# lbrndnr/LBAudioDetective

Hardware: AMD Instinct MI355X
Metric: audio_seconds_fingerprinted_per_sec (higher is better)
Workload: dtype f32; 1 GPU; configs[1]: 100k synthetic 1 s @44.1 kHz mono clips, 1024-pt FFT, stride 64, fingerprint-only, input resident in HBM; one step = 10 passes over the batch; clips_per_gpu=100000, samples_per_clip=44100, window=1024, stride=64, bands=32, subfingerprints_per_clip=5, kernel_variant=0, parallelism=clips sharded x1, no collective

## Files before the change

lbaudiodetective_amd/csrc/api_detective.cpp:

```cpp
#include "internal.hpp"

#include <new>
#include "audiofile.hpp"

#include <cmath>
#include <cstdlib>
#include <cstring>

namespace lbad {

uint64_t subfingerprint_count(uint64_t n_samples, uint32_t window, uint32_t stride) {
    if (stride == 0 || n_samples < window) return 0;
    return ((n_samples - window) / stride) / kRowsPerFrame;
}

static bool valid_window(uint32_t w) { return w >= kMinWindow && w <= kMaxWindow && (w & (w - 1)) == 0; }

static void free_plan(Plan& p) {
    if (p.d_tw) (void)hipFree(p.d_tw);
    if (p.d_bands) (void)hipFree(p.d_bands);
    if (p.d_bin_const) (void)hipFree(p.d_bin_const);
    if (p.d_claim) (void)hipFree(p.d_claim);
    p = Plan();
}

static OSStatus plan_kernels(Plan& p) {
    p.pruned_ok = rows_pruned_supported(p);
    if (p.pruned_ok && !p.d_bin_const) {
        std::vector<float> bc;
        rows_pruned_constants(bc);
        LBAD_HIP(hipMalloc(reinterpret_cast<void**>(&p.d_bin_const), bc.size() * sizeof(float)));
        LBAD_HIP(hipMemcpy(p.d_bin_const, bc.data(), bc.size() * sizeof(float), hipMemcpyHostToDevice));
    }
    p.full_ok = rows_full_supported(p);
    p.stream_ok = rows_stream_supported(p);
    p.stream2_ok = rows_stream2_supported(p);
    if ((p.full_ok || p.stream_ok || p.stream2_ok) && !p.d_claim) LBAD_HIP(hipMalloc(reinterpret_cast<void**>(&p.d_claim), 8 * sizeof(uint32_t)));
    return noErr;
}

OSStatus ensure_plan(LBAudioDetective* d) {
    const double rate = d->format.mSampleRate;
    if (!valid_window(d->window) || d->stride == 0 || d->bands == 0 || d->bands > kMaxBands || !(rate > 0.0) ||
        d->subfp_len == 0 || d->subfp_len > LBAD_MAX_SUBFINGERPRINT_LENGTH ||
        d->subfp_len > kRowsPerFrame * d->bands)
        return kLBAudioDetectiveArgumentInvalid;
    Plan& p = d->plan;
    p.tune_waves = d->tune_waves;
    p.tune_cache = d->tune_cache;
    if (p.valid && p.sample_rate == rate && p.window == d->window && p.bands == d->bands && p.subfp_len == d->subfp_len) {
        if (p.stride == d->stride) return noErr;
        p.stride = d->stride;
        p.valid = false;
        OSStatus st = plan_kernels(p);
        if (st != noErr) return st;
        p.valid = true;
        return noErr;
    }
    if (!device_ready()) return kLBAudioDetectiveDeviceUnavailable;
    free_plan(p);
    p.tune_waves = d->tune_waves;
    p.tune_cache = d->tune_cache;
    p.sample_rate = rate;
    p.window = d->window;
    p.stride = d->stride;
    p.bands = d->bands;
    p.subfp_len = d->subfp_len;
    p.log2w = 0;
    while ((1u << p.log2w) < p.window) ++p.log2w;
    p.keep = (p.subfp_len + 1) / 2;
    make_band_table(rate, p.window, p.bands, p.table);
    std::vector<float> re, im;
    make_twiddles(p.window, re, im);
    const size_t half = p.window / 2;
    LBAD_HIP(hipMalloc(reinterpret_cast<void**>(&p.d_tw), 2 * half * sizeof(float)));
    LBAD_HIP(hipMemcpy(p.d_tw, re.data(), half * sizeof(float), hipMemcpyHostToDevice));
    LBAD_HIP(hipMemcpy(p.d_tw + half, im.data(), half * sizeof(float), hipMemcpyHostToDevice));
    plan_sparse(p);
    std::vector<uint32_t> tbl(8 * (size_t)p.bands + 1);
    for (uint32_t b = 0; b < p.bands; ++b) {
        tbl[b] = p.table.lo[b];
        tbl[p.bands + b] = p.table.hi[b];
        const float div = (float)(p.table.indices[b + 1] - p.table.indices[b]);
        std::memcpy(&tbl[2 * p.bands + b], &div, 4);
        tbl[3 * p.bands + b] = p.bands;
        tbl[4 * p.bands + b] = b;
        uint32_t mult = 0, off = 0xFFFFFFFFu;
        if (p.sparse.ok) {
            const uint32_t pos = b >= 16 ? p.sparse.pos_right[b - 16] : (b == p.sparse.left ? p.sparse.pos_left : 0xFFu);
            if (pos != 0xFFu) { mult = p.sparse.n_stored; off = pos; }
        }
        tbl[5 * p.bands + b] = mult;
        tbl[6 * p.bands + b] = off;
        tbl[7 * p.bands + b] = p.table.term_at[b];
    }
    tbl[8 * (size_t)p.bands] = p.table.term_end;
    LBAD_HIP(hipMalloc(reinterpret_cast<void**>(&p.d_bands), tbl.size() * sizeof(uint32_t)));
    LBAD_HIP(hipMemcpy(p.d_bands, tbl.data(), tbl.size() * sizeof(uint32_t), hipMemcpyHostToDevice));
    OSStatus st = plan_kernels(p);
    if (st != noErr) return st;
    p.valid = true;
    return noErr;
}

static OSStatus ensure_scratch(LBAudioDetective* d, uint64_t floats) {
    if (d->d_frames_cap >= floats) return noErr;
    if (d->d_frames) (void)hipFree(d->d_frames);
    d->d_frames = nullptr;
    d->d_frames_cap = 0;
    LBAD_HIP(hipMalloc(reinterpret_cast<void**>(&d->d_frames), floats * sizeof(float)));
    d->d_frames_cap = floats;
    return noErr;
}

static hipError_t apply_file_tail(const Plan& p, const FileTail& t, const void* d_pcm, uint64_t rows_total, float* frames,
                                  hipStream_t stream) {
    if (t.mode == 3) return launch_empty_rows_batch(p, t.d_files, t.n_files, t.max_rows, frames, stream);
    const uint64_t rows = t.rows ? t.rows : rows_total;
    if (t.first_short >= rows) return hipSuccess;
    float* file_frames = frames + t.row_begin * p.bands;
    if (t.mode == 1)
        return launch_empty_rows(p, file_frames + t.first_short * p.bands, rows - t.first_short, stream);
    if (t.mode == 2)
        return launch_file_tail(p, static_cast<const float*>(d_pcm) + t.pcm_begin, t.n_client, p.stride, t.first_short,
                                (uint32_t)(rows - t.first_short), t.d_tbl, file_frames, stream);
    return hipSuccess;
}

struct StreamOrder {
    LBAudioDetective* d;
    hipStream_t stream;
    bool active = false;
    hipError_t begin() {
        hipStreamCaptureStatus cap = hipStreamCaptureStatusNone;
        if (hipStreamIsCapturing(stream, &cap) != hipSuccess) { (void)hipGetLastError(); return hipSuccess; }
        if (cap != hipStreamCaptureStatusNone) return hipSuccess;
        if (!d->done) {
            hipError_t e = hipEventCreateWithFlags(&d->done, hipEventDisableTiming);
            if (e != hipSuccess) return e;
        }
        active = true;
        if (d->done_valid && d->done_stream != stream) return hipStreamWaitEvent(stream, d->done, 0);
        return hipSuccess;
    }
    ~StreamOrder() {
        if (!active) return;
        d->done_valid = hipEventRecord(d->done, stream) == hipSuccess;
        d->done_stream = stream;
    }
};

OSStatus fingerprint_clips_device(LBAudioDetective* d, const void* d_pcm_raw, uint32_t fmt, uint64_t n_clips,
                                  uint64_t spc, uint32_t* d_packed, float* d_raw, float* d_haar, hipStream_t stream,
                                  const FileTail* tail, size_t n_tails) {
    if (fmt > 2) return kLBAudioDetectiveArgumentInvalid;
    if (tail && (n_clips != 1 || fmt != 0)) return kLBAudioDetectiveArgumentInvalid;
    LBAD_LOCK(d);
    const size_t elem = fmt == 1 ? 2 : 4;
    const char* d_pcm = static_cast<const char*>(d_pcm_raw);
    OSStatus st = ensure_plan(d);
    if (st != noErr) return st;
    const Plan& p = d->plan;
    const uint64_t per = subfingerprint_count(spc, p.window, p.stride);
    if (per == 0 || n_clips == 0) return noErr;
    if (per > 0xFFFFFFFFull / kRowsPerFrame) return kLBAudioDetectiveArgumentInvalid;
    const bool pairs_ok = reinterpret_cast<uintptr_t>(d_pcm_raw) % (2 * elem) == 0 && ((spc & 1) == 0 || n_clips == 1);
    const bool stream_ok = p.stream_ok && pairs_ok;
    const bool stream2_ok = p.stream2_ok && pairs_ok && d->variant != 3;
    const bool full_ok = p.full_ok && rows_full_supported_fmt(p, fmt);
    bool special = p.pruned_ok || full_ok || stream_ok || stream2_ok;
    if (d->variant == 3) {
        if (!full_ok && !p.pruned_ok) return kLBAudioDetectiveArgumentInvalid;
    }
    if (d->variant == 1) special = false;
    if (d->variant >= 2 && !special) return kLBAudioDetectiveArgumentInvalid;
    StreamOrder order{d, stream};
    LBAD_HIP(order.begin());
    const bool special2 = d->variant != 1 && haar_select32_supported(p);
    const bool compact = special && p.pruned_ok && special2 && p.sparse.ok && !tail && !d_raw && d->variant != 4;
    auto stage1 = [&](const void* pcm_in, uint64_t nc, float* frames_out) -> hipError_t {
        if (special && p.pruned_ok)
            return launch_rows_pruned(p, p.d_bin_const, pcm_in, fmt, nc, spc, (uint32_t)per, frames_out, stream, compact);
        if (special && stream2_ok) return launch_rows_stream2(p, pcm_in, fmt, nc, spc, (uint32_t)per, frames_out, stream);
        if (special && full_ok) return launch_rows_full(p, pcm_in, fmt, nc, spc, (uint32_t)per, frames_out, stream);
        if (special) return launch_rows_stream(p, pcm_in, fmt, nc, spc, (uint32_t)per, frames_out, stream);
        return launch_fft_bands(p, pcm_in, fmt, nc, spc, (uint32_t)per, frames_out, stream);
    };
    auto stage2 = [&](float* frames_in, uint64_t nf, uint32_t* packed_out, float* haar_out) -> hipError_t {
        if (compact && haar_out) {
            hipError_t e = hipMemsetAsync(haar_out, 0, nf * kRowsPerFrame * p.bands * sizeof(float), stream);
            if (e != hipSuccess) return e;
        }
        return special2 ? launch_haar_select32(p, frames_in, nf, packed_out, haar_out, stream, compact)
                        : launch_haar_select(p, frames_in, nf, packed_out, haar_out, stream);
    };
    const uint64_t frame_floats = (uint64_t)kRowsPerFrame * p.bands;
    if (d_raw) {
        LBAD_HIP(stage1(d_pcm, n_clips, d_raw));
        for (size_t t = 0; tail && t < n_tails; ++t) LBAD_HIP(apply_file_tail(p, tail[t], d_pcm, per * kRowsPerFrame, d_raw, stream));
        LBAD_HIP(stage2(d_raw, n_clips * per, d_packed, d_haar));
        return noErr;
    }
    uint64_t chunk = (d->scratch_limit / sizeof(float)) / (per * frame_floats);
    if (chunk == 0) chunk = 1;
    if (chunk > n_clips) chunk = n_clips;
    st = ensure_scratch(d, chunk * per * frame_floats);
    if (st != noErr) return st;
    auto mark = [&]() -> hipError_t {
        if (!d->timing) return hipSuccess;
        if (d->ev_used == d->ev.size()) {
            hipEvent_t e;
            hipError_t err = hipEventCreate(&e);
            if (err != hipSuccess) return err;
            d->ev.push_back(e);
        }
        return hipEventRecord(d->ev[d->ev_used++], stream);
    };
    for (uint64_t c0 = 0; c0 < n_clips; c0 += chunk) {
        const uint64_t nc = (n_clips - c0) < chunk ? (n_clips - c0) : chunk;
        LBAD_HIP(mark());
        LBAD_HIP(stage1(d_pcm + c0 * spc * elem, nc, d->d_frames));
        for (size_t t = 0; tail && t < n_tails; ++t)
            LBAD_HIP(apply_file_tail(p, tail[t], d_pcm, per * kRowsPerFrame, d->d_frames, stream));
        LBAD_HIP(mark());
        LBAD_HIP(stage2(d->d_frames, nc * per, d_packed + c0 * per * kPackedWords,
                        d_haar ? d_haar + c0 * per * frame_floats : nullptr));
        LBAD_HIP(mark());
    }
    return noErr;
}

constexpr size_t kPinnedLimit = 512u << 10;

OSStatus grow_device(void** ptr, size_t* cap, size_t bytes) {
    if (*cap >= bytes) return noErr;
    if (*ptr) (void)hipFree(*ptr);
    *ptr = nullptr;
    *cap = 0;
    const size_t want = bytes + bytes / 4;
    LBAD_HIP(hipMalloc(ptr, want));
    *cap = want;
    return noErr;
}

static OSStatus ensure_io(LBAudioDetective* d, size_t pcm_bytes, size_t packed_bytes, size_t extra_bytes) {
    OSStatus st = grow_device(&d->d_io_pcm, &d->d_io_pcm_cap, pcm_bytes + extra_bytes + 256);
    if (st != noErr) return st;
// ... 751 lines not shown
```

lbaudiodetective_amd/csrc/k_haar_select32.hip:

```cpp
#include "internal.hpp"

#include <type_traits>

namespace lbad {
namespace {

constexpr uint32_t kCand = 128;
constexpr int kChunkDw = 20;

constexpr uint32_t kFastDivLo = 0x0D800000u;
constexpr uint32_t kFastDivHi = 0x7E800000u;

struct DivGuard {
    uint32_t lo = 0xFFFFFFFFu, hi = 0u;
    __device__ __forceinline__ void dividends(float a, float b) {
        lo = min(lo, min((__float_as_uint(a) << 1) - 1u, (__float_as_uint(b) << 1) - 1u));
    }
    __device__ __forceinline__ void inputs(float a, float b) {
        hi = max(hi, max(__float_as_uint(a) & 0x7fffffffu, __float_as_uint(b) & 0x7fffffffu));
    }
    __device__ __forceinline__ bool bad() const { return lo < 2u * kFastDivLo - 1u || hi > kFastDivHi; }
};

template <bool FAST>
__device__ __forceinline__ float div_c(float x, float d, float r) {
    if constexpr (FAST) {
        const float q0 = __fmul_rn(x, r);
        const float e = __fmaf_rn(-d, q0, x);
        return __fmaf_rn(e, r, q0);
    } else {
        return __fdiv_rn(x, d);
    }
}

constexpr uint32_t kHistBuckets = 2048;

__device__ __forceinline__ uint32_t wave_prefix_sum(uint32_t x) {
    x += (uint32_t)__builtin_amdgcn_update_dpp(0, (int)x, 0x111 , 0xF, 0xF, false);
    x += (uint32_t)__builtin_amdgcn_update_dpp(0, (int)x, 0x112 , 0xF, 0xF, false);
    x += (uint32_t)__builtin_amdgcn_update_dpp(0, (int)x, 0x114 , 0xF, 0xF, false);
    x += (uint32_t)__builtin_amdgcn_update_dpp(0, (int)x, 0x118 , 0xF, 0xF, false);
    x += (uint32_t)__builtin_amdgcn_update_dpp(0, (int)x, 0x142 , 0xA, 0xF, false);
    x += (uint32_t)__builtin_amdgcn_update_dpp(0, (int)x, 0x143 , 0xC, 0xF, false);
    return x;
}

template <int WAVES>
__device__ __forceinline__ uint32_t slots_sum(const uint32_t* slot) {
    uint32_t c = 0;
#pragma unroll
    for (int w = 0; w < WAVES; ++w) c += slot[w];
    return c;
}

template <int WAVES>
__device__ __forceinline__ uint32_t block_sum(uint32_t v, uint32_t* s_red, int parity) {
#pragma unroll
    for (int off = 32; off > 0; off >>= 1) v += __shfl_xor(v, off, 64);
    uint32_t* slot = s_red + 8 * parity;
    if ((threadIdx.x & 63) == 0) slot[threadIdx.x >> 6] = v;
    __syncthreads();
    return slots_sum<WAVES>(slot);
}

constexpr uint32_t kLightLo = 0x25800000u;
typedef float f2 __attribute__((ext_vector_type(2)));

struct LightGuard {
    uint32_t lo_in = 0xFFFFFFFFu, lo_4 = 0xFFFFFFFFu;
    float hi = 0.0f;
    __device__ __forceinline__ void levels34(f2 a, f2 b, f2 c) {
        auto t = [](float x) { return (__float_as_uint(x) << 1) - 1u; };
        lo_4 = min(min(min(t(a.x), t(a.y)), min(t(b.x), t(b.y))), min(t(c.x), t(c.y)));
    }
    __device__ __forceinline__ bool bad(float s4) const {
        return lo_in < 2u * kLightLo - 1u || lo_4 < 2u * kFastDivLo - 1u || !(hi <= __uint_as_float(kFastDivHi)) || s4 != s4;
    }
};

template <bool FAST>
__device__ __forceinline__ float haar16_impl(const float (&in)[16], float (&d)[15], float root, float r_root,
                                             float root2, float r_root2, DivGuard& g) {
    float a[16];
#pragma unroll
    for (int i = 0; i < 16; i += 2) {
        if constexpr (FAST) {
            g.inputs(in[i], in[i + 1]);
            g.dividends(in[i], in[i + 1]);
        }
        a[i] = div_c<FAST>(in[i], root, r_root);
        a[i + 1] = div_c<FAST>(in[i + 1], root, r_root);
    }
    auto bfly = [&](float x, float y, float& sum, float& dif) {
        const float sp = __fadd_rn(x, y), sm = __fsub_rn(x, y);
        if constexpr (FAST) g.dividends(sp, sm);
        sum = div_c<FAST>(sp, root2, r_root2);
        dif = div_c<FAST>(sm, root2, r_root2);
    };
    float s1[8], s2[4], s3[2], s4;
#pragma unroll
    for (int i = 0; i < 8; ++i) bfly(a[2 * i], a[2 * i + 1], s1[i], d[i]);
#pragma unroll
    for (int i = 0; i < 4; ++i) bfly(s1[2 * i], s1[2 * i + 1], s2[i], d[8 + i]);
#pragma unroll
    for (int i = 0; i < 2; ++i) bfly(s2[2 * i], s2[2 * i + 1], s3[i], d[12 + i]);
    bfly(s3[0], s3[1], s4, d[14]);
    return s4;
}


struct DivConst {
    unsigned long long r, nd;
    __device__ __forceinline__ explicit DivConst(float d)
        : r(__builtin_amdgcn_readfirstlane(__float_as_uint(__fdiv_rn(1.0f, d)))),
          nd(__builtin_amdgcn_readfirstlane(__float_as_uint(-d))) {}
};

__device__ __forceinline__ void pk_prescale8(f2 (&x)[8], f2 (&q)[8], const DivConst& c) {
    asm("v_pk_mul_f32 %0, %8, %[r] op_sel_hi:[1,0]\n"
        "v_pk_mul_f32 %1, %9, %[r] op_sel_hi:[1,0]\n"
        "v_pk_mul_f32 %2, %10, %[r] op_sel_hi:[1,0]\n"
        "v_pk_mul_f32 %3, %11, %[r] op_sel_hi:[1,0]\n"
        "v_pk_mul_f32 %4, %12, %[r] op_sel_hi:[1,0]\n"
        "v_pk_mul_f32 %5, %13, %[r] op_sel_hi:[1,0]\n"
        "v_pk_mul_f32 %6, %14, %[r] op_sel_hi:[1,0]\n"
        "v_pk_mul_f32 %7, %15, %[r] op_sel_hi:[1,0]\n"
        "v_pk_fma_f32 %8, %0, %[nd], %8 op_sel_hi:[1,0,1]\n"
        "v_pk_fma_f32 %9, %1, %[nd], %9 op_sel_hi:[1,0,1]\n"
        "v_pk_fma_f32 %10, %2, %[nd], %10 op_sel_hi:[1,0,1]\n"
        "v_pk_fma_f32 %11, %3, %[nd], %11 op_sel_hi:[1,0,1]\n"
        "v_pk_fma_f32 %12, %4, %[nd], %12 op_sel_hi:[1,0,1]\n"
        "v_pk_fma_f32 %13, %5, %[nd], %13 op_sel_hi:[1,0,1]\n"
        "v_pk_fma_f32 %14, %6, %[nd], %14 op_sel_hi:[1,0,1]\n"
        "v_pk_fma_f32 %15, %7, %[nd], %15 op_sel_hi:[1,0,1]\n"
        "v_pk_fma_f32 %0, %8, %[r], %0 op_sel_hi:[1,0,1]\n"
        "v_pk_fma_f32 %1, %9, %[r], %1 op_sel_hi:[1,0,1]\n"
        "v_pk_fma_f32 %2, %10, %[r], %2 op_sel_hi:[1,0,1]\n"
        "v_pk_fma_f32 %3, %11, %[r], %3 op_sel_hi:[1,0,1]\n"
        "v_pk_fma_f32 %4, %12, %[r], %4 op_sel_hi:[1,0,1]\n"
        "v_pk_fma_f32 %5, %13, %[r], %5 op_sel_hi:[1,0,1]\n"
        "v_pk_fma_f32 %6, %14, %[r], %6 op_sel_hi:[1,0,1]\n"
        "v_pk_fma_f32 %7, %15, %[r], %7 op_sel_hi:[1,0,1]\n"
        "s_nop 0"
        : "=&v"(q[0]), "=&v"(q[1]), "=&v"(q[2]), "=&v"(q[3]), "=&v"(q[4]), "=&v"(q[5]), "=&v"(q[6]), "=&v"(q[7]),
          "+v"(x[0]), "+v"(x[1]), "+v"(x[2]), "+v"(x[3]), "+v"(x[4]), "+v"(x[5]), "+v"(x[6]), "+v"(x[7])
        : [r] "s"(c.r), [nd] "s"(c.nd));
}

__device__ __forceinline__ void pk_level1(f2 (&p)[8], f2 (&q)[8], const DivConst& c) {
    asm("v_pk_add_f32 %8, %8, %8 op_sel:[0,1] op_sel_hi:[0,1] neg_hi:[0,1]\n"
        "v_pk_add_f32 %9, %9, %9 op_sel:[0,1] op_sel_hi:[0,1] neg_hi:[0,1]\n"
        "v_pk_add_f32 %10, %10, %10 op_sel:[0,1] op_sel_hi:[0,1] neg_hi:[0,1]\n"
        "v_pk_add_f32 %11, %11, %11 op_sel:[0,1] op_sel_hi:[0,1] neg_hi:[0,1]\n"
        "v_pk_add_f32 %12, %12, %12 op_sel:[0,1] op_sel_hi:[0,1] neg_hi:[0,1]\n"
        "v_pk_add_f32 %13, %13, %13 op_sel:[0,1] op_sel_hi:[0,1] neg_hi:[0,1]\n"
        "v_pk_add_f32 %14, %14, %14 op_sel:[0,1] op_sel_hi:[0,1] neg_hi:[0,1]\n"
        "v_pk_add_f32 %15, %15, %15 op_sel:[0,1] op_sel_hi:[0,1] neg_hi:[0,1]\n"
        "v_pk_mul_f32 %0, %8, %[r] op_sel_hi:[1,0]\n"
        "v_pk_mul_f32 %1, %9, %[r] op_sel_hi:[1,0]\n"
        "v_pk_mul_f32 %2, %10, %[r] op_sel_hi:[1,0]\n"
        "v_pk_mul_f32 %3, %11, %[r] op_sel_hi:[1,0]\n"
        "v_pk_mul_f32 %4, %12, %[r] op_sel_hi:[1,0]\n"
        "v_pk_mul_f32 %5, %13, %[r] op_sel_hi:[1,0]\n"
        "v_pk_mul_f32 %6, %14, %[r] op_sel_hi:[1,0]\n"
        "v_pk_mul_f32 %7, %15, %[r] op_sel_hi:[1,0]\n"
        "v_pk_fma_f32 %8, %0, %[nd], %8 op_sel_hi:[1,0,1]\n"
        "v_pk_fma_f32 %9, %1, %[nd], %9 op_sel_hi:[1,0,1]\n"
        "v_pk_fma_f32 %10, %2, %[nd], %10 op_sel_hi:[1,0,1]\n"
        "v_pk_fma_f32 %11, %3, %[nd], %11 op_sel_hi:[1,0,1]\n"
        "v_pk_fma_f32 %12, %4, %[nd], %12 op_sel_hi:[1,0,1]\n"
        "v_pk_fma_f32 %13, %5, %[nd], %13 op_sel_hi:[1,0,1]\n"
        "v_pk_fma_f32 %14, %6, %[nd], %14 op_sel_hi:[1,0,1]\n"
        "v_pk_fma_f32 %15, %7, %[nd], %15 op_sel_hi:[1,0,1]\n"
        "v_pk_fma_f32 %0, %8, %[r], %0 op_sel_hi:[1,0,1]\n"
        "v_pk_fma_f32 %1, %9, %[r], %1 op_sel_hi:[1,0,1]\n"
        "v_pk_fma_f32 %2, %10, %[r], %2 op_sel_hi:[1,0,1]\n"
        "v_pk_fma_f32 %3, %11, %[r], %3 op_sel_hi:[1,0,1]\n"
        "v_pk_fma_f32 %4, %12, %[r], %4 op_sel_hi:[1,0,1]\n"
        "v_pk_fma_f32 %5, %13, %[r], %5 op_sel_hi:[1,0,1]\n"
        "v_pk_fma_f32 %6, %14, %[r], %6 op_sel_hi:[1,0,1]\n"
        "v_pk_fma_f32 %7, %15, %[r], %7 op_sel_hi:[1,0,1]\n"
        "s_nop 0"
        : "=&v"(q[0]), "=&v"(q[1]), "=&v"(q[2]), "=&v"(q[3]), "=&v"(q[4]), "=&v"(q[5]), "=&v"(q[6]), "=&v"(q[7]),
          "+v"(p[0]), "+v"(p[1]), "+v"(p[2]), "+v"(p[3]), "+v"(p[4]), "+v"(p[5]), "+v"(p[6]), "+v"(p[7])
        : [r] "s"(c.r), [nd] "s"(c.nd));
}
// ... 677 lines not shown
```

lbaudiodetective_amd/csrc/k_rows_pruned.hip:

```cpp
#include "internal.hpp"
#include "fft64_lane.hpp"

namespace lbad {
namespace {

constexpr int kW = 1024;
constexpr int kStride = 64;
constexpr int kBands = 32;
constexpr int kBins = 22;
constexpr int kRows = 43;
constexpr int kRowsA = 22;
constexpr int kRowDw = 20;
constexpr int kWinDw = 464;
constexpr int kWaves = 4;
constexpr int kThreads = kWaves * 64;
constexpr int kUnitWindows = 32;
constexpr int kSpan = (kUnitWindows - 1) * kStride + kW;
constexpr int kSpanDw = kSpan + 16 * (kSpan >> 6);
constexpr int kTDw = kWaves * 8 * kWinDw;
constexpr int kBinConst = 14;
constexpr int kConstStride = 20;
constexpr int kConstDw = kBins * kConstStride;
constexpr int kClaimOffset = 312;
constexpr int kLdsBytes = (kSpanDw + kTDw + kConstDw + 4) * 4;
constexpr int kWgPerCu = 2;
static_assert(kWgPerCu * kLdsBytes <= 160 * 1024, "two workgroups must fit one CU's LDS");

using namespace lane64;

template <int I>
__device__ __forceinline__ cplx stage6_row(const cplx (&x)[64]) {
    constexpr int j = I < 22 ? I : I - 11;
    constexpr bool plus = I < 22;
    const cplx u = x[j], v = x[j + 32];
    if constexpr (j == 0) {
        return u + v;
    } else if constexpr (j == 16) {
        return plus ? fma2(mk(1.0f, -1.0f), v.yx, u) : fma2(mk(-1.0f, 1.0f), v.yx, u);
    } else {
        constexpr float wr = kTw64Re[j], wi = kTw64Im[j];
        if constexpr (plus) return fma2(mk(wr, wr), v, fma2(mk(-wi, wi), v.yx, u));
        else return fma2(mk(-wr, -wr), v, fma2(mk(wi, -wi), v.yx, u));
    }
}

template <int I, int END, int FIRST>
__device__ __forceinline__ void store_rows(const cplx (&x)[64], float* trow) {
    if constexpr (I < END) {
        *(lds_vf32x2*)(trow + (I - FIRST) * kRowDw) = stage6_row<I>(x);
        store_rows<I + 1, END, FIRST>(x, trow);
    }
}

template <int I, int END, int FIRST>
__device__ __forceinline__ void hold_rows(const cplx (&x)[64], cplx (&h)[kRows - kRowsA]) {
    if constexpr (I < END) {
        h[I - FIRST] = stage6_row<I>(x);
        hold_rows<I + 1, END, FIRST>(x, h);
    }
}
template <int I, int N>
__device__ __forceinline__ void store_held(const cplx (&h)[kRows - kRowsA], float* trow) {
    if constexpr (I < N) {
        *(lds_vf32x2*)(trow + I * kRowDw) = h[I];
        store_held<I + 1, N>(h, trow);
    }
}

template <int M>
__device__ __forceinline__ void load_points(cplx (&x)[64], const float* src) {
    if constexpr (M < 64) {
        constexpr int m = brev6(M);
        x[M] = *(const lds_vf32x2*)(src + (m & 3) * 16 + (m >> 2) * 80);
        load_points<M + 1>(x, src);
    }
}

struct TreeIn {
    float4 q0, q1, q2, q3;
};
struct TreeTw {
    f32x2 t0, t1, t2;
};
__device__ __forceinline__ TreeIn tree_load(const float* row) {
    TreeIn in;
    in.q0 = *reinterpret_cast<const float4*>(row);
    in.q1 = *reinterpret_cast<const float4*>(row + 4);
    in.q2 = *reinterpret_cast<const float4*>(row + 8);
    in.q3 = *reinterpret_cast<const float4*>(row + 12);
    return in;
}
__device__ __forceinline__ TreeTw tree_twiddles(const float* tw) {
    TreeTw t;
    t.t0 = *reinterpret_cast<const f32x2*>(tw);
    t.t1 = *reinterpret_cast<const f32x2*>(tw + 2);
    t.t2 = *reinterpret_cast<const f32x2*>(tw + 4);
    return t;
}
__device__ __forceinline__ cplx tree_eval(const TreeIn& in, const TreeTw& t) {
    const cplx x0 = mk(in.q0.x, in.q0.y), x1 = mk(in.q0.z, in.q0.w), x2 = mk(in.q1.x, in.q1.y), x3 = mk(in.q1.z, in.q1.w);
    const cplx x4 = mk(in.q2.x, in.q2.y), x5 = mk(in.q2.z, in.q2.w), x6 = mk(in.q3.x, in.q3.y), x7 = mk(in.q3.z, in.q3.w);
    const cplx y0 = madd(x0, t.t0.x, t.t0.y, x4), y1 = madd(x1, t.t0.x, t.t0.y, x5);
    const cplx y2 = madd(x2, t.t0.x, t.t0.y, x6), y3 = madd(x3, t.t0.x, t.t0.y, x7);
    const cplx z0 = madd(y0, t.t1.x, t.t1.y, y2), z1 = madd(y1, t.t1.x, t.t1.y, y3);
    return madd(z0, t.t2.x, t.t2.y, z1);
}

typedef __attribute__((address_space(1))) const void gvoid_t;
typedef __attribute__((address_space(3))) void lvoid_t;

template <int FMT>
__device__ __forceinline__ void span_to_lds(const void* __restrict__ pcm_raw, uint64_t first, float* span, int wave,
                                            int lane) {
    if constexpr (FMT == 0) {
        const float* src = static_cast<const float*>(pcm_raw) + first + lane + 64 * wave;
        float* dst = span + 80 * wave;
        constexpr int kFull = (kSpan / 64) / kWaves;
#pragma unroll
        for (int i = 0; i < kFull; ++i)
            __builtin_amdgcn_global_load_lds((gvoid_t*)(src + 64 * kWaves * i), (lvoid_t*)(dst + 80 * kWaves * i), 4, 0, 0);
        if (wave < kSpan / 64 - kFull * kWaves)
            __builtin_amdgcn_global_load_lds((gvoid_t*)(src + 64 * kWaves * kFull), (lvoid_t*)(dst + 80 * kWaves * kFull), 4, 0, 0);
    } else if constexpr (FMT == 1) {
        const int16_t* src = static_cast<const int16_t*>(pcm_raw) + first;
        for (int s = threadIdx.x; s < kSpan; s += kThreads)
            span[s + 16 * (s >> 6)] = (float)src[s] * (1.0f / 32768.0f);
    } else {
        const int32_t* src = static_cast<const int32_t*>(pcm_raw) + first;
        for (int s = threadIdx.x; s < kSpan; s += kThreads)
            span[s + 16 * (s >> 6)] = (float)src[s] * (1.0f / 2147483648.0f);
    }
}

template <int FMT>
__global__ __launch_bounds__(kThreads, kWgPerCu) void frame_rows_pruned_kernel(const void* __restrict__ pcm_raw,
                                                                         uint64_t samples_per_clip,
                                                                         uint32_t frames_per_clip, uint64_t n_units,
                                                                         uint64_t units_per_xcd,
                                                                         const float* __restrict__ bin_const,
                                                                         const uint32_t* __restrict__ band_tbl,
                                                                         uint32_t* __restrict__ claim_ctr,
                                                                         float* __restrict__ frames, uint32_t frame_dw,
                                                                         uint32_t place_tbl) {
    extern __shared__ __attribute__((aligned(16))) float smem[];
    float* span = smem;
    const int wave = __builtin_amdgcn_readfirstlane(threadIdx.x >> 6);
    const int lane = threadIdx.x & 63;
    float* tbuf = smem + kSpanDw + wave * (8 * kWinDw);
    float* vbuf = tbuf;
    float* cbuf = smem + kSpanDw + kTDw;
    uint32_t* claim_slot = reinterpret_cast<uint32_t*>(cbuf + kConstDw);

    const uint32_t wg_per_xcd = gridDim.x >> 3;
    const uint64_t xcd_begin = (uint64_t)(blockIdx.x & 7) * units_per_xcd;
    const uint64_t xcd_end = xcd_begin + units_per_xcd < n_units ? xcd_begin + units_per_xcd : n_units;
    uint64_t unit = xcd_begin + 4 * (uint64_t)(blockIdx.x >> 3);
    if (unit >= xcd_end) return;

    auto span_start = [&](uint64_t u) {
        const uint32_t frame = (uint32_t)(u >> 2);
        const uint32_t clip = frame / frames_per_clip;
        const uint32_t fi = frame - clip * frames_per_clip;
        return (uint64_t)clip * samples_per_clip + (uint64_t)(fi * 128 + (uint32_t)(u & 3) * kUnitWindows) * kStride;
    };
    uint32_t* my_ctr = claim_ctr + (blockIdx.x & 7);
    const bool claimer = threadIdx.x == 0;
    uint32_t claimed = 0;

    span_to_lds<FMT>(pcm_raw, span_start(unit), span, wave, lane);
    for (int i = threadIdx.x; i < kBins * kBinConst; i += kThreads)
        cbuf[(i / kBinConst) * kConstStride + (i % kBinConst)] = bin_const[i];
    const int band = lane & 31;
    const uint32_t b_lo = band_tbl[band], b_hi = band_tbl[kBands + band];
    const float b_div = __uint_as_float(band_tbl[2 * kBands + band]);
    const uint32_t b_mult = band_tbl[place_tbl * kBands + band], b_off = band_tbl[(place_tbl + 1) * kBands + band];

    const int w8 = lane >> 3, r = lane & 7;
    const float inv_norm = 1.0f / (float)(kW / 4);
#ifdef LBAD_EXP_TREE_NOSWAP
    const int rr = r;
#else
    const int rr = r ^ ((((w8 + 1) >> 1) & 1) << 2);
#endif
    int tk[3];
#pragma unroll
    for (int rd = 0; rd < 3; ++rd) tk[rd] = rr + 8 * rd < kBins ? rr + 8 * rd : kBins - 1;
    const bool last_valid = rr + 16 < kBins;

    __syncthreads();
    TreeTw twp[3], twm[3];
    f32x2 ws[3];
#pragma unroll
    for (int rd = 0; rd < 3; ++rd) {
        const float* c = cbuf + tk[rd] * kConstStride;
        twp[rd] = tree_twiddles(c);
        twm[rd] = tree_twiddles(c + 6);
        ws[rd] = *reinterpret_cast<const f32x2*>(c + 12);
    }

    float out[4] = {0.0f, 0.0f, 0.0f, 0.0f};
    float* out_ptr = nullptr;
#ifdef LBAD_EXP_TIMELINE
    long long ts[8];
#define STAMP(i) ts[i] = __builtin_readcyclecounter()
#else
#define STAMP(i)
#endif
    for (;;) {
        STAMP(0);
#ifdef LBAD_EXP_TIMELINE
        const unsigned long long rt0 = __builtin_amdgcn_s_memrealtime();
#endif
        __builtin_amdgcn_s_waitcnt(0x0F70);
        const uint32_t quarter = (uint32_t)(unit & 3);
        if (quarter == 3 && claimer) claim_slot[0] = claimed;
        __syncthreads();
        STAMP(1);

        cplx x[64];
        load_points<0>(x, span + 80 * (8 * wave + w8) + 2 * r);
        const uint64_t next = quarter == 3 ? xcd_begin + 4 * ((uint64_t)wg_per_xcd + claim_slot[0]) : unit + 1;
        __syncthreads();
        if (next < xcd_end) span_to_lds<FMT>(pcm_raw, span_start(next), span, wave, lane);
        if (quarter == 0 && claimer) claimed = atomicAdd(my_ctr, 1u);
#ifndef LBAD_EXP_TIMELINE
        if (out_ptr) {
#pragma unroll
            for (int q = 0; q < 4; ++q) out_ptr[q * 2 * b_mult] = out[q];
        }
#endif
        STAMP(2);

        __builtin_amdgcn_s_setprio(0);
        stage_blocks<1, 0>(x);
        stage_blocks<2, 0>(x);
        stage_blocks<3, 0>(x);
        stage_blocks<4, 0>(x);
        stage_blocks<5, 0>(x);
        STAMP(3);
        __builtin_amdgcn_s_setprio(3);

        store_rows<0, kRowsA, 0>(x, tbuf + w8 * kWinDw + 2 * r);
        cplx held[kRows - kRowsA];
        hold_rows<kRowsA, kRows, kRowsA>(x, held);
        cplx za[3];
        {
            TreeIn in[3];
#pragma unroll
            for (int rd = 0; rd < 3; ++rd) in[rd] = tree_load(tbuf + w8 * kWinDw + tk[rd] * kRowDw);
            store_held<0, kRows - kRowsA>(held, tbuf + w8 * kWinDw + 2 * r);
#pragma unroll
            for (int rd = 0; rd < 3; ++rd) za[rd] = tree_eval(in[rd], twp[rd]);
        }
        STAMP(4);
        float pw[3];
        {
            TreeIn in[3];
#pragma unroll
            for (int rd = 0; rd < 3; ++rd) {
                const int k = tk[rd];
                in[rd] = tree_load(tbuf + w8 * kWinDw + (21 - k) * kRowDw);
            }
#pragma unroll
            for (int rd = 0; rd < 3; ++rd) {
                const int k = tk[rd];
                const cplx b = tree_eval(in[rd], twm[rd]);
                const cplx a = za[rd];
                float re, im;
                if (k == 0) {
                    const float sm = a.x + a.y, df = a.x - a.y;
                    re = sm + sm;
                    im = df + df;
                } else {
                    const float sr = a.x + b.x, si = a.y - b.y;
                    const float dr = a.x - b.x, di = a.y + b.y;
                    const float wr = ws[rd].x, wi = ws[rd].y;
                    re = __fmaf_rn(wr, di, __fmaf_rn(wi, dr, sr));
                    im = __fmaf_rn(-wr, dr, __fmaf_rn(wi, di, si));
                }
                if (re > 0.0f) re = __fmul_rn(re, inv_norm);
                if (im > 0.0f) im = __fmul_rn(im, inv_norm);
                pw[rd] = __fadd_rn(__fmul_rn(re, re), __fmul_rn(im, im));
            }
        }
        STAMP(5);
#pragma unroll
        for (int rd = 0; rd < 3; ++rd)
            if (rd < 2 || last_valid) vbuf[w8 * 24 + tk[rd]] = pw[rd];

        float p[4] = {0.0f, 0.0f, 0.0f, 0.0f};
        const float* vb = vbuf + (lane >> 5) * 24;
        for (uint32_t k = b_lo; k < b_hi; ++k) {
            float v[4];
#pragma unroll
            for (int q = 0; q < 4; ++q) v[q] = vb[q * 48 + k];
#pragma unroll
            for (int q = 0; q < 4; ++q)
                if (v[q] == v[q] && fabsf(v[q]) != INFINITY) p[q] = __fadd_rn(p[q], v[q]);
        }
#pragma unroll
        for (int q = 0; q < 4; ++q) out[q] = __fdiv_rn(p[q], b_div);
        out_ptr = b_off != 0xFFFFFFFFu
                      ? frames + (unit >> 2) * frame_dw + (quarter * kUnitWindows + 8 * wave + (lane >> 5)) * b_mult + b_off
                      : nullptr;
#ifdef LBAD_EXP_TIMELINE
        STAMP(6);
        if (lane == 0) {
            float* o = frames + ((unit >> 2) * 128 + quarter * kUnitWindows + 8 * wave) * kBands;
            for (int i = 1; i < 7; ++i) o[i - 1] = (float)(ts[i] - ts[i - 1]);
            o[6] = (float)(ts[0] & 0xFFFFFF);
            o[7] = (float)__builtin_amdgcn_s_getreg(((16 - 1) << 11) | 4);
            o[8] = (float)(ts[0] >> 24 & 0xFFFFFF);
            o[9] = (float)(__builtin_amdgcn_s_memrealtime() - rt0);
        }
#endif
        if (next >= xcd_end) break;
        unit = next;
    }
#ifndef LBAD_EXP_TIMELINE
    if (out_ptr) {
#pragma unroll
        for (int q = 0; q < 4; ++q) out_ptr[q * 2 * b_mult] = out[q];
    }
#endif
}

}

bool rows_pruned_supported(const Plan& p) {
    if (p.window != (uint32_t)kW || p.stride != (uint32_t)kStride || p.bands != (uint32_t)kBands) return false;
    if (p.table.kmax > (uint32_t)kBins) return false;
    std::vector<float> re, im;
    make_twiddles(kW, re, im);
    for (int t = 0; t < 32; ++t)
        if (re[16 * t] != kTw64Re[t] || im[16 * t] != kTw64Im[t]) return false;
    return true;
}

void rows_pruned_constants(std::vector<float>& out) {
    std::vector<float> re, im;
    make_twiddles(kW, re, im);
    out.assign((size_t)kClaimOffset + 8, 0.0f);
    for (int k = 0; k < kBins; ++k) {
        float* c = &out[(size_t)k * kBinConst];
        c[0] = re[8 * k]; c[1] = im[8 * k];
        c[2] = re[4 * k]; c[3] = im[4 * k];
        c[4] = re[2 * k]; c[5] = im[2 * k];
        if (k > 0) {
            c[6] = -re[8 * (64 - k)];   c[7] = -im[8 * (64 - k)];
            c[8] = -re[4 * (128 - k)];  c[9] = -im[4 * (128 - k)];
            c[10] = -re[2 * (256 - k)]; c[11] = -im[2 * (256 - k)];
            c[12] = re[k]; c[13] = im[k];
        }
    }
}

template <int FMT>
static hipError_t launch_rows_fmt(const Plan& plan, const float* d_bin_const, const void* d_pcm, uint64_t n_frames,
                                  uint64_t samples_per_clip, uint32_t frames_per_clip, float* d_frames,
                                  hipStream_t stream, bool compact) {
    static PerDevice attr;
    if (attr.changed(kLdsBytes)) {
        hipError_t e = hipFuncSetAttribute(reinterpret_cast<const void*>(frame_rows_pruned_kernel<FMT>),
                                           hipFuncAttributeMaxDynamicSharedMemorySize, kLdsBytes);
        if (e != hipSuccess) return e;
    }
    const uint64_t n_units = n_frames * 4, units_per_xcd = 4 * ((n_frames + 7) / 8);
    const int n_cu = device_cu_count();
    uint64_t wg_per_xcd = ((uint64_t)n_cu * kWgPerCu + 7) / 8;
    if (wg_per_xcd > units_per_xcd / 4) wg_per_xcd = units_per_xcd / 4;
    uint32_t* claim = reinterpret_cast<uint32_t*>(const_cast<float*>(d_bin_const)) + kClaimOffset;
    hipError_t e = hipMemsetAsync(claim, 0, 8 * sizeof(uint32_t), stream);
    if (e != hipSuccess) return e;
    hipLaunchKernelGGL(frame_rows_pruned_kernel<FMT>, dim3((uint32_t)(wg_per_xcd * 8)), dim3(kThreads), kLdsBytes,
                       stream, d_pcm, samples_per_clip, frames_per_clip, n_units, units_per_xcd, d_bin_const,
                       plan.d_bands, claim, d_frames, compact ? plan.sparse.frame_dw() : 128u * kBands, compact ? 5u : 3u);
    return hipGetLastError();
}

hipError_t launch_rows_pruned(const Plan& plan, const float* d_bin_const, const void* d_pcm, uint32_t fmt,
                              uint64_t n_clips, uint64_t samples_per_clip, uint32_t frames_per_clip, float* d_frames,
                              hipStream_t stream, bool compact) {
    if (compact && !plan.sparse.ok) return hipErrorInvalidValue;
    const uint64_t n_frames = n_clips * frames_per_clip;
    if (n_frames == 0) return hipSuccess;
    if (n_frames > 0x7fffffffull) return hipErrorInvalidValue;
    if (n_frames * 4 + 8 > 0x7fffffffull) return hipErrorInvalidValue;
    switch (fmt) {
        case 0: return launch_rows_fmt<0>(plan, d_bin_const, d_pcm, n_frames, samples_per_clip, frames_per_clip, d_frames, stream, compact);
        case 1: return launch_rows_fmt<1>(plan, d_bin_const, d_pcm, n_frames, samples_per_clip, frames_per_clip, d_frames, stream, compact);
        case 2: return launch_rows_fmt<2>(plan, d_bin_const, d_pcm, n_frames, samples_per_clip, frames_per_clip, d_frames, stream, compact);
        default: return hipErrorInvalidValue;
    }
}

}
```

Measured before the change: 5.378 million audio-s/s.

## Use guarded reciprocal band division, self-resetting claim counters, and scalar span loads

```diff
diff --git a/lbaudiodetective_amd/csrc/api_detective.cpp b/lbaudiodetective_amd/csrc/api_detective.cpp
--- a/lbaudiodetective_amd/csrc/api_detective.cpp
+++ b/lbaudiodetective_amd/csrc/api_detective.cpp
@@ -1,4 +1,5 @@
 #include "internal.hpp"
+#include "const_div.hpp"
 
 #include <new>
 #include "audiofile.hpp"
@@ -77,7 +78,7 @@
     LBAD_HIP(hipMemcpy(p.d_tw, re.data(), half * sizeof(float), hipMemcpyHostToDevice));
     LBAD_HIP(hipMemcpy(p.d_tw + half, im.data(), half * sizeof(float), hipMemcpyHostToDevice));
     plan_sparse(p);
-    std::vector<uint32_t> tbl(8 * (size_t)p.bands + 1);
+    std::vector<uint32_t> tbl(11 * (size_t)p.bands);
     for (uint32_t b = 0; b < p.bands; ++b) {
         tbl[b] = p.table.lo[b];
         tbl[p.bands + b] = p.table.hi[b];
@@ -93,6 +94,9 @@
         tbl[5 * p.bands + b] = mult;
         tbl[6 * p.bands + b] = off;
         tbl[7 * p.bands + b] = p.table.term_at[b];
+        const float rcp = 1.0f / div;
+        std::memcpy(&tbl[9 * p.bands + b], &rcp, 4);
+        tbl[10 * p.bands + b] = band_div_proven(div) ? 1u : 0u;
     }
     tbl[8 * (size_t)p.bands] = p.table.term_end;
     LBAD_HIP(hipMalloc(reinterpret_cast<void**>(&p.d_bands), tbl.size() * sizeof(uint32_t)));
diff --git a/lbaudiodetective_amd/csrc/band_div_proven.inc b/lbaudiodetective_amd/csrc/band_div_proven.inc
--- /dev/null
+++ b/lbaudiodetective_amd/csrc/band_div_proven.inc
@@ -0,0 +1,8 @@
+1, 2, 3, 4, 5, 6, 7, 8, 9, 10, 11, 12, 13, 14, 15, 16,
+17, 18, 19, 20, 21, 22, 23, 24, 25, 26, 27, 28, 29, 30, 31, 32,
+33, 34, 35, 36, 37, 38, 39, 40, 41, 42, 43, 44, 45, 46, 47, 48,
+49, 50, 51, 52, 53, 54, 55, 56, 57, 58, 59, 60, 61, 62, 63, 64,
+65, 66, 67, 68, 69, 70, 71, 72, 73, 74, 75, 76, 77, 78, 79, 80,
+81, 82, 83, 84, 85, 86, 87, 88, 89, 90, 91, 92, 93, 94, 95, 96,
+97, 98, 99, 100, 101, 102, 103, 104, 105, 106, 107, 108, 109, 110, 111, 112,
+113, 114, 115, 116, 117, 118, 119, 120, 121, 122, 123, 124, 125, 126, 127, 128,
diff --git a/lbaudiodetective_amd/csrc/const_div.hpp b/lbaudiodetective_amd/csrc/const_div.hpp
--- /dev/null
+++ b/lbaudiodetective_amd/csrc/const_div.hpp
@@ -0,0 +1,45 @@
+#pragma once
+#include <cstdint>
+
+namespace lbad {
+
+constexpr uint32_t kFastDivLo = 0x0D800000u;
+constexpr uint32_t kFastDivHi = 0x7E800000u;
+
+constexpr uint32_t kBandDivLo = kFastDivLo;
+constexpr uint32_t kBandDivHi = 0x7F7FFFFFu;
+
+inline bool band_div_proven(float d) {
+    static const uint32_t proven[] = {
+#include "band_div_proven.inc"
+    };
+    for (uint32_t v : proven)
+        if (d == (float)v) return true;
+    return false;
+}
+
+#ifdef __HIPCC__
+struct DivGuard {
+    uint32_t lo = 0xFFFFFFFFu, hi = 0u;
+    __device__ __forceinline__ void dividends(float a, float b) {
+        lo = min(lo, min((__float_as_uint(a) << 1) - 1u, (__float_as_uint(b) << 1) - 1u));
+    }
+    __device__ __forceinline__ void inputs(float a, float b) {
+        hi = max(hi, max(__float_as_uint(a) & 0x7fffffffu, __float_as_uint(b) & 0x7fffffffu));
+    }
+    __device__ __forceinline__ bool bad() const { return lo < 2u * kFastDivLo - 1u || hi > kFastDivHi; }
+};
+
+template <bool FAST>
+__device__ __forceinline__ float div_c(float x, float d, float r) {
+    if constexpr (FAST) {
+        const float q0 = __fmul_rn(x, r);
+        const float e = __fmaf_rn(-d, q0, x);
+        return __fmaf_rn(e, r, q0);
+    } else {
+        return __fdiv_rn(x, d);
+    }
+}
+#endif
+
+}
diff --git a/lbaudiodetective_amd/csrc/k_haar_select32.hip b/lbaudiodetective_amd/csrc/k_haar_select32.hip
--- a/lbaudiodetective_amd/csrc/k_haar_select32.hip
+++ b/lbaudiodetective_amd/csrc/k_haar_select32.hip
@@ -1,4 +1,5 @@
 #include "internal.hpp"
+#include "const_div.hpp"
 
 #include <type_traits>
 
@@ -8,30 +9,6 @@
 constexpr uint32_t kCand = 128;
 constexpr int kChunkDw = 20;
 
-constexpr uint32_t kFastDivLo = 0x0D800000u;
-constexpr uint32_t kFastDivHi = 0x7E800000u;
-
-struct DivGuard {
-    uint32_t lo = 0xFFFFFFFFu, hi = 0u;
-    __device__ __forceinline__ void dividends(float a, float b) {
-        lo = min(lo, min((__float_as_uint(a) << 1) - 1u, (__float_as_uint(b) << 1) - 1u));
-    }
-    __device__ __forceinline__ void inputs(float a, float b) {
-        hi = max(hi, max(__float_as_uint(a) & 0x7fffffffu, __float_as_uint(b) & 0x7fffffffu));
-    }
-    __device__ __forceinline__ bool bad() const { return lo < 2u * kFastDivLo - 1u || hi > kFastDivHi; }
-};
-
-template <bool FAST>
-__device__ __forceinline__ float div_c(float x, float d, float r) {
-    if constexpr (FAST) {
-        const float q0 = __fmul_rn(x, r);
-        const float e = __fmaf_rn(-d, q0, x);
-        return __fmaf_rn(e, r, q0);
-    } else {
-        return __fdiv_rn(x, d);
-    }
-}
 
 constexpr uint32_t kHistBuckets = 2048;
 
diff --git a/lbaudiodetective_amd/csrc/k_rows_pruned.hip b/lbaudiodetective_amd/csrc/k_rows_pruned.hip
--- a/lbaudiodetective_amd/csrc/k_rows_pruned.hip
+++ b/lbaudiodetective_amd/csrc/k_rows_pruned.hip
@@ -1,4 +1,5 @@
 #include "internal.hpp"
+#include "const_div.hpp"
 #include "fft64_lane.hpp"
 
 namespace lbad {
@@ -22,6 +23,7 @@
 constexpr int kConstStride = 20;
 constexpr int kConstDw = kBins * kConstStride;
 constexpr int kClaimOffset = 312;
+constexpr int kClaimWords = 16;
 constexpr int kLdsBytes = (kSpanDw + kTDw + kConstDw + 4) * 4;
 constexpr int kWgPerCu = 2;
 static_assert(kWgPerCu * kLdsBytes <= 160 * 1024, "two workgroups must fit one CU's LDS");
@@ -113,14 +115,25 @@
 __device__ __forceinline__ void span_to_lds(const void* __restrict__ pcm_raw, uint64_t first, float* span, int wave,
                                             int lane) {
     if constexpr (FMT == 0) {
-        const float* src = static_cast<const float*>(pcm_raw) + first + lane + 64 * wave;
-        float* dst = span + 80 * wave;
+        const uint64_t first_w = first + 64 * wave;
+        const uint64_t first_s = ((uint64_t)__builtin_amdgcn_readfirstlane((uint32_t)(first_w >> 32)) << 32) |
+                                 (uint32_t)__builtin_amdgcn_readfirstlane((uint32_t)first_w);
+        const char* src = static_cast<const char*>(pcm_raw) + 4 * first_s;
+        const uint32_t lane_off = 4u * (uint32_t)lane;
+        uint32_t lbase = (uint32_t)(size_t)(lvoid_t*)(span + 80 * wave);
+        int tail_wave = wave;
+        asm volatile("" : "+s"(lbase), "+s"(tail_wave));
         constexpr int kFull = (kSpan / 64) / kWaves;
-#pragma unroll
-        for (int i = 0; i < kFull; ++i)
-            __builtin_amdgcn_global_load_lds((gvoid_t*)(src + 64 * kWaves * i), (lvoid_t*)(dst + 80 * kWaves * i), 4, 0, 0);
-        if (wave < kSpan / 64 - kFull * kWaves)
-            __builtin_amdgcn_global_load_lds((gvoid_t*)(src + 64 * kWaves * kFull), (lvoid_t*)(dst + 80 * kWaves * kFull), 4, 0, 0);
+        static_assert(kFull == 11, "three groups of four loads");
+#define LBAD_SPAN_LOAD(I)                                                                                            \
+    __builtin_amdgcn_global_load_lds((gvoid_t*)(src + 4 * 64 * kWaves * ((I) & ~3) + lane_off),                      \
+                                     (lvoid_t*)(size_t)(lbase + 4 * (80 * kWaves * (I) - 64 * kWaves * ((I) & 3))),  \
+                                     4, 4 * 64 * kWaves * ((I) & 3), 0)
+        LBAD_SPAN_LOAD(0); LBAD_SPAN_LOAD(1); LBAD_SPAN_LOAD(2); LBAD_SPAN_LOAD(3);
+        LBAD_SPAN_LOAD(4); LBAD_SPAN_LOAD(5); LBAD_SPAN_LOAD(6); LBAD_SPAN_LOAD(7);
+        LBAD_SPAN_LOAD(8); LBAD_SPAN_LOAD(9); LBAD_SPAN_LOAD(10);
+        if (tail_wave < kSpan / 64 - kFull * kWaves) LBAD_SPAN_LOAD(11);
+#undef LBAD_SPAN_LOAD
     } else if constexpr (FMT == 1) {
         const int16_t* src = static_cast<const int16_t*>(pcm_raw) + first;
         for (int s = threadIdx.x; s < kSpan; s += kThreads)
@@ -129,6 +142,16 @@
         const int32_t* src = static_cast<const int32_t*>(pcm_raw) + first;
         for (int s = threadIdx.x; s < kSpan; s += kThreads)
             span[s + 16 * (s >> 6)] = (float)src[s] * (1.0f / 2147483648.0f);
+    }
+}
+
+__device__ __forceinline__ void claims_done(uint32_t* claim_ctr) {
+    __threadfence();
+    if (atomicAdd(claim_ctr + 8, 1u) == gridDim.x - 1u) {
+        __threadfence();
+#pragma unroll
+        for (int i = 0; i < 9; ++i) atomicExch(claim_ctr + i, 0u);
+        __threadfence();
     }
 }
 
@@ -155,7 +178,10 @@
     const uint64_t xcd_begin = (uint64_t)(blockIdx.x & 7) * units_per_xcd;
     const uint64_t xcd_end = xcd_begin + units_per_xcd < n_units ? xcd_begin + units_per_xcd : n_units;
     uint64_t unit = xcd_begin + 4 * (uint64_t)(blockIdx.x >> 3);
-    if (unit >= xcd_end) return;
+    if (unit >= xcd_end) {
+        if (threadIdx.x == 0) claims_done(claim_ctr);
+        return;
+    }
 
     auto span_start = [&](uint64_t u) {
         const uint32_t frame = (uint32_t)(u >> 2);
@@ -164,6 +190,7 @@
         return (uint64_t)clip * samples_per_clip + (uint64_t)(fi * 128 + (uint32_t)(u & 3) * kUnitWindows) * kStride;
     };
     uint32_t* my_ctr = claim_ctr + (blockIdx.x & 7);
+    asm volatile("" : "+v"(my_ctr));
     const bool claimer = threadIdx.x == 0;
     uint32_t claimed = 0;
 
@@ -173,6 +200,8 @@
     const int band = lane & 31;
     const uint32_t b_lo = band_tbl[band], b_hi = band_tbl[kBands + band];
     const float b_div = __uint_as_float(band_tbl[2 * kBands + band]);
+    const float b_rcp = __uint_as_float(band_tbl[9 * kBands + band]);
+    const int b_fast_hi = band_tbl[10 * kBands + band] ? (int)kBandDivHi : -1;
     const uint32_t b_mult = band_tbl[place_tbl * kBands + band], b_off = band_tbl[(place_tbl + 1) * kBands + band];
 
     const int w8 = lane >> 3, r = lane & 7;
@@ -298,8 +327,18 @@
             for (int q = 0; q < 4; ++q)
                 if (v[q] == v[q] && fabsf(v[q]) != INFINITY) p[q] = __fadd_rn(p[q], v[q]);
         }
-#pragma unroll
-        for (int q = 0; q < 4; ++q) out[q] = __fdiv_rn(p[q], b_div);
+        DivGuard g;
+        g.dividends(p[0], p[1]);
+        g.dividends(p[2], p[3]);
+        const int p_max = max(max((int)__float_as_uint(p[0]), (int)__float_as_uint(p[1])),
+                              max((int)__float_as_uint(p[2]), (int)__float_as_uint(p[3])));
+        if (__builtin_expect(__builtin_amdgcn_ballot_w64(g.lo < 2u * kBandDivLo - 1u || p_max > b_fast_hi) == 0, 1)) {
+#pragma unroll
+            for (int q = 0; q < 4; ++q) out[q] = div_c<true>(p[q], b_div, b_rcp);
+        } else {
+#pragma unroll
+            for (int q = 0; q < 4; ++q) out[q] = div_c<false>(p[q], b_div, b_rcp);
+        }
         out_ptr = b_off != 0xFFFFFFFFu
                       ? frames + (unit >> 2) * frame_dw + (quarter * kUnitWindows + 8 * wave + (lane >> 5)) * b_mult + b_off
                       : nullptr;
@@ -323,6 +362,7 @@
         for (int q = 0; q < 4; ++q) out_ptr[q * 2 * b_mult] = out[q];
     }
 #endif
+    if (claimer) claims_done(claim_ctr);
 }
 
 }
@@ -340,7 +380,7 @@
 void rows_pruned_constants(std::vector<float>& out) {
     std::vector<float> re, im;
     make_twiddles(kW, re, im);
-    out.assign((size_t)kClaimOffset + 8, 0.0f);
+    out.assign((size_t)kClaimOffset + kClaimWords, 0.0f);
     for (int k = 0; k < kBins; ++k) {
         float* c = &out[(size_t)k * kBinConst];
         c[0] = re[8 * k]; c[1] = im[8 * k];
@@ -370,8 +410,6 @@
     uint64_t wg_per_xcd = ((uint64_t)n_cu * kWgPerCu + 7) / 8;
     if (wg_per_xcd > units_per_xcd / 4) wg_per_xcd = units_per_xcd / 4;
     uint32_t* claim = reinterpret_cast<uint32_t*>(const_cast<float*>(d_bin_const)) + kClaimOffset;
-    hipError_t e = hipMemsetAsync(claim, 0, 8 * sizeof(uint32_t), stream);
-    if (e != hipSuccess) return e;
     hipLaunchKernelGGL(frame_rows_pruned_kernel<FMT>, dim3((uint32_t)(wg_per_xcd * 8)), dim3(kThreads), kLdsBytes,
                        stream, d_pcm, samples_per_clip, frames_per_clip, n_units, units_per_xcd, d_bin_const,
                        plan.d_bands, claim, d_frames, compact ? plan.sparse.frame_dw() : 128u * kBands, compact ? 5u : 3u);
```

Result: faster. 5.434 million audio-s/s (median of 6 runs) (+1.0%).
